# ctlab/metafast

Hardware: AMD Instinct MI355X
Metric: k-mers/s counted+graphed at k=31, 150 bp reads (higher is better)
Workload: dtype u64

## Files before the change

### metafast_amd/csrc/mf_skm.hip

```cpp
#include "mf_common.h"
#include "mf_count_dev.h"
#include <algorithm>
#include <memory>
#include <vector>

typedef ulonglong2 skm_rec;
typedef uint32_t skm_v4 __attribute__((ext_vector_type(4)));
#define SKM_LINE 4
#define SKM_QCAP 16
#define SKM_DIGIT_BITS 22
#define SKM_CT 512
#define SKM_NW (SKM_CT / 64)

__device__ __forceinline__ bool skm_rec_valid(const skm_rec &r) { return ((uint32_t)r.y & 63u) != 63u; }
__device__ __forceinline__ uint32_t skm_rec_n(const skm_rec &r) { return (uint32_t)r.y & 63u; }
__device__ __forceinline__ uint32_t skm_rec_digits(const skm_rec &r) { return (uint32_t)(r.y >> 6) & ((1u << SKM_DIGIT_BITS) - 1u); }

template <int K> struct skm_word {
    static constexpr int W = K - mf_skm_m(K) + 1;
    static constexpr int NM = 31 + W;
    static constexpr int RMAX = (MF_SKM_BASES - (K - 1)) < 20 ? (MF_SKM_BASES - (K - 1)) : 20;
    uint32_t D[4];
    uint32_t mh[32];
    uint32_t valid;
// ... 71 lines not shown
    const uint64_t b0 = w * 32;
    const uint4 *p = reinterpret_cast<const uint4 *>(bases + (b0 < n_bases ? b0 : 0));
    const bool in1 = b0 + 16 < n_bases;
    const uint4 c0 = p[0], c1 = p[in1 ? 1 : 0];
    S.D[0] = b0 < n_bases ? mf_dec16(c0) : 0u; S.D[1] = in1 ? mf_dec16(c1) : 0u;
    S.D[2] = skm_from_next_lane(S.D[0]); S.D[3] = skm_from_next_lane(S.D[1]);
    S.valid = m;
    static_assert(64 - M - 31 >= 16, "reversed words");
    const uint32_t R3 = skm_rc16(S.D[0]);
    const uint32_t R[4] = {0u, skm_from_next_lane(R3), skm_rc16(S.D[1]), R3};
    uint32_t hs[34];
#pragma unroll
    for (int i = 0; i < 32; i++) {
        const uint32_t f = skm_mmer_at<M>(S.D, i), r = skm_mmer_at<M>(R, 64 - M - i);
        hs[i] = mf_mmer_hash(f < r ? f : r, M);
    }
    constexpr int W = skm_word<K>::W;
    static_assert(W >= 3 && W <= 18, "window");
    static_assert(NM <= 64, "halo");
    auto min3 = [](uint32_t a, uint32_t b, uint32_t c) { const uint32_t m = a < b ? a : b; return m < c ? m : c; };
    hs[32] = skm_from_next_lane(hs[0]); hs[33] = skm_from_next_lane(hs[1]);
    uint32_t a[38];
#pragma unroll
    for (int i = 0; i < 32; i++) a[i] = min3(hs[i], hs[i + 1], hs[i + 2]);
    if (W >= 9) {
        uint32_t b[32 + 9];
#pragma unroll
        for (int i = 32; i < 38; i++) a[i] = skm_from_next_lane(a[i - 32]);
#pragma unroll
        for (int i = 0; i < 32; i++) b[i] = min3(a[i], a[i + 3], a[i + 6]);
#pragma unroll
        for (int i = 32; i < 32 + W - 9; i++) b[i] = skm_from_next_lane(b[i - 32]);
#pragma unroll
        for (int j = 0; j < 32; j++) S.mh[j] = b[j] < b[j + W - 9] ? b[j] : b[j + W - 9];
    } else {
        constexpr int D = W - 3 < 3 ? W - 3 : 3;
#pragma unroll
        for (int i = 32; i < 32 + W - 3; i++) a[i] = skm_from_next_lane(a[i - 32]);
#pragma unroll
        for (int j = 0; j < 32; j++) S.mh[j] = min3(a[j], a[j + D], a[j + W - 3]);
    }
    skm_cut_mask<K>(S, m);
}

__device__ __forceinline__ uint32_t skm_sel(uint32_t a, uint32_t b, unsigned long long m) {
    uint32_t r;
    asm("v_cndmask_b32 %0, %1, %2, %3" : "=v"(r) : "v"(a), "v"(b), "s"(m));
    return r;
}
template <int K>
__device__ __forceinline__ uint32_t skm_mh_at(const skm_word<K> &S, uint32_t s) {
    uint32_t a[16], b[8], c[4], d[2];
    const unsigned long long s0 = __ballot((s & 1u) != 0), s1 = __ballot((s & 2u) != 0), s2 = __ballot((s & 4u) != 0),
                             s3 = __ballot((s & 8u) != 0), s4 = __ballot((s & 16u) != 0);
#pragma unroll
    for (int i = 0; i < 16; i++) a[i] = skm_sel(S.mh[2 * i], S.mh[2 * i + 1], s0);
#pragma unroll
    for (int i = 0; i < 8; i++) b[i] = skm_sel(a[2 * i], a[2 * i + 1], s1);
#pragma unroll
    for (int i = 0; i < 4; i++) c[i] = skm_sel(b[2 * i], b[2 * i + 1], s2);
#pragma unroll
    for (int i = 0; i < 2; i++) d[i] = skm_sel(c[2 * i], c[2 * i + 1], s3);
    return skm_sel(d[0], d[1], s4);
}

template <int K>
__device__ __forceinline__ void skm_next_run(const skm_word<K> &S, uint32_t &cut, uint32_t &s, uint32_t &len) {
    s = (uint32_t)__builtin_ctz(cut);
    cut &= cut - 1u;
    const uint32_t stop = (cut | ~S.valid) & ~((2u << s) - 1u);
    const uint32_t e = stop ? (uint32_t)__builtin_ctz(stop) : 32u;
    len = e - s;
    if (len > (uint32_t)skm_word<K>::RMAX) { len = (uint32_t)skm_word<K>::RMAX; cut |= 1u << (s + len); }
}

template <int K>
__device__ __forceinline__ skm_rec skm_make_rec(const uint32_t (&D)[4], uint32_t s, uint32_t len, uint32_t digits, uint32_t D4 = 0u) {
    const uint32_t o = (2u * s) & 31u;
    const unsigned long long q = __ballot(s >= 16u);
    const uint32_t E0 = skm_sel(D[0], D[1], q), E1 = skm_sel(D[1], D[2], q), E2 = skm_sel(D[2], D[3], q), E3 = skm_sel(D[3], D4, q), E4 = skm_sel(D4, 0u, q);
    uint32_t T0 = E0, T1 = E1, T2 = E2, T3 = E3;
    if (o) {
        T0 = __builtin_amdgcn_alignbit(E0, E1, 32u - o);
        T1 = __builtin_amdgcn_alignbit(E1, E2, 32u - o);
        T2 = __builtin_amdgcn_alignbit(E2, E3, 32u - o);
        T3 = __builtin_amdgcn_alignbit(E3, E4, 32u - o);
    }
    static_assert(K >= 17 && K <= 32, "the first dword is kept whole");
    const int kb = 2 * (int)(len + K - 1);
    const uint64_t m01 = (uint64_t)((int64_t)0x8000000000000000ull >> ((kb < 64 ? kb : 64) - 1));
    const uint64_t m23 = ~(~0ull >> (kb > 64 ? kb - 64 : 0));
    T1 &= (uint32_t)m01; T2 &= (uint32_t)(m23 >> 32); T3 &= (uint32_t)m23;
    skm_rec r;
    r.x = ((uint64_t)T0 << 32) | T1;
    r.y = ((uint64_t)T2 << 32) | (uint64_t)(T3 & 0xF0000000u) | ((uint64_t)digits << 6) | (uint64_t)len;
    return r;
}
__device__ __forceinline__ void skm_route(uint32_t mh, int bits1, uint32_t &d1, uint32_t &digits) {
    const uint32_t ph = mf_remix32(mh);
    d1 = bits1 ? ph >> (32 - bits1) : 0u;
    digits = (bits1 ? (ph << bits1) : ph) >> (32 - SKM_DIGIT_BITS);
}

template <int K>
__global__ __launch_bounds__(1024) void k_skm_hist(const uint8_t *__restrict__ bases, uint64_t n_bases, const uint32_t *__restrict__ vmask,
                                                   uint64_t n_words, uint64_t words_per_block, int bits1,
                                                   uint32_t *__restrict__ blockhist, uint32_t *__restrict__ blockocc, int G, int stride,
                                                   uint32_t dlo, uint32_t dhi) {
    extern __shared__ __attribute__((aligned(16))) unsigned char smem[];
    const int nd = 1 << bits1;
    uint32_t *hist = reinterpret_cast<uint32_t *>(smem), *occ = hist + nd;
    for (int i = threadIdx.x; i < 2 * nd; i += blockDim.x) hist[i] = 0;
    __syncthreads();
    const uint64_t wlo = (uint64_t)blockIdx.x * words_per_block;
    const uint64_t whi = wlo + words_per_block < n_words ? wlo + words_per_block : n_words;
    for (uint64_t wb = wlo; wb < whi; wb += (uint64_t)blockDim.x * (uint64_t)stride) {
        const uint64_t w = wb + threadIdx.x;
        const uint32_t m = w < whi ? vmask[w] : 0u;
        if (__ballot(m != 0u) == 0ull) continue;
        skm_word<K> S;
        skm_scan_word<K>(S, bases, n_bases, w < n_words ? w : 0, m);
        uint32_t cut = S.cut;
        while (__ballot(cut != 0u) != 0ull) {
            if (cut) {
                uint32_t s, len, d1, digits;
                skm_next_run<K>(S, cut, s, len);
                skm_route(skm_mh_at<K>(S, s), bits1, d1, digits);
                if (d1 >= dlo && d1 < dhi) {
                    atomicAdd(&hist[d1], 1u);
                    if (blockocc) atomicAdd(&occ[d1], len);
                }
            }
        }
    }
    __syncthreads();
    for (int i = threadIdx.x; i < nd; i += blockDim.x) {
        blockhist[(size_t)i * G + blockIdx.x] = hist[i];
        if (blockocc) blockocc[(size_t)i * G + blockIdx.x] = occ[i];
    }
}

struct skm_stage {
    skm_rec *line;
    uint64_t *cur;
    uint64_t *q_pos;
    uint32_t *ctr;
    uint32_t *q_d;
    int nd;
};
__device__ __forceinline__ skm_stage skm_stage_carve(unsigned char *smem, int nd) {
    skm_stage L;
    L.nd = nd;
    L.line = reinterpret_cast<skm_rec *>(smem);
    L.cur = reinterpret_cast<uint64_t *>(L.line + (size_t)nd * SKM_LINE + 64);
    L.q_pos = L.cur + nd;
    L.ctr = reinterpret_cast<uint32_t *>(L.q_pos + 16 * SKM_QCAP);
    L.q_d = L.ctr + nd + 64;
    return L;
}
__host__ __device__ static inline size_t skm_stage_bytes(int nd) {
    return ((size_t)nd * SKM_LINE + 64) * 16 + (size_t)nd * 8 + 16 * SKM_QCAP * 8 + ((size_t)nd + 64) * 4 + 16 * SKM_QCAP * 4;
}
__device__ __forceinline__ void skm_lds_write4_add_rtn4(const uint32_t (&wa)[4], const skm_v4 (&wv)[4], const uint32_t (&a)[4],
                                                        const uint32_t (&inc)[4], uint32_t (&old)[4]) {
    asm volatile("ds_write_b128 %4, %8\n\tds_write_b128 %5, %9\n\tds_write_b128 %6, %10\n\tds_write_b128 %7, %11\n\t"
                 "ds_add_rtn_u32 %0, %12, %16\n\tds_add_rtn_u32 %1, %13, %17\n\tds_add_rtn_u32 %2, %14, %18\n\t"
                 "ds_add_rtn_u32 %3, %15, %19\n\ts_waitcnt lgkmcnt(0)"
                 : "=&v"(old[0]), "=&v"(old[1]), "=&v"(old[2]), "=&v"(old[3])
                 : "v"(wa[0]), "v"(wa[1]), "v"(wa[2]), "v"(wa[3]), "v"(wv[0]), "v"(wv[1]), "v"(wv[2]), "v"(wv[3]),
                   "v"(a[0]), "v"(a[1]), "v"(a[2]), "v"(a[3]), "v"(inc[0]), "v"(inc[1]), "v"(inc[2]), "v"(inc[3])
                 : "memory");
}
#define SKM_CH 256
#define SKM_NONE (~0ull)
struct skm_dyn {
    unsigned long long *gcur;
    const uint64_t *rend;
    unsigned int *overflow;
    uint64_t dump;
    unsigned long long *save;
};
template <bool DYN>
__device__ __forceinline__ uint64_t skm_take_line(const skm_stage &L, uint32_t dg, const skm_dyn &Dy) {
    uint64_t pos = L.cur[dg];
    if (DYN && (pos == SKM_NONE || (pos & (uint64_t)(SKM_CH - 1)) == 0ull)) {
        pos = atomicAdd(&Dy.gcur[dg], (unsigned long long)SKM_CH);
        if (pos + SKM_CH > Dy.rend[dg]) { atomicExch(Dy.overflow, 1u); pos = Dy.dump; }
    }
    L.cur[dg] = pos + SKM_LINE;
    return pos;
}
template <bool DYN = false>
__device__ __forceinline__ void skm_stage_insert(const skm_stage &L, skm_rec *__restrict__ out, const uint32_t (&d)[4],
                                                 const skm_rec (&rec)[4], bool (&pending)[4], const skm_dyn &Dy = skm_dyn()) {
    const uint32_t ctr0 = mf_lds_addr(L.ctr), line0 = mf_lds_addr(L.line);
    const uint32_t dummy_ctr = ctr0 + 4u * ((uint32_t)L.nd + (uint32_t)mf_lane());
    const uint32_t dummy_slot = line0 + 16u * ((uint32_t)L.nd * SKM_LINE + (uint32_t)mf_lane());
    skm_v4 wv[4];
#pragma unroll
    for (int b = 0; b < 4; b++) { wv[b].x = (uint32_t)rec[b].x; wv[b].y = (uint32_t)(rec[b].x >> 32); wv[b].z = (uint32_t)rec[b].y; wv[b].w = (uint32_t)(rec[b].y >> 32); }
    for (;;) {
        bool any = false;
#pragma unroll
        for (int b = 0; b < 4; b++) any |= pending[b];
        if (__ballot(any) == 0ull) break;
        uint32_t ca[4], w[4], inc[4], old[4], old2[4], wa[4];
        bool got[4];
#pragma unroll
        for (int b = 0; b < 4; b++) ca[b] = pending[b] ? ctr0 + 4u * d[b] : dummy_ctr;
        mf_lds_read4(ca, w);
#pragma unroll
        for (int b = 0; b < 4; b++) inc[b] = (pending[b] && (w[b] & 0xFFFFu) < (uint32_t)SKM_LINE) ? 1u : 0u;
        mf_lds_add_rtn4(ca, inc, old);
#pragma unroll
        for (int b = 0; b < 4; b++) {
            got[b] = inc[b] && (old[b] & 0xFFFFu) < (uint32_t)SKM_LINE;
            wa[b] = got[b] ? line0 + 16u * (d[b] * SKM_LINE + (old[b] & 0xFFFFu)) : dummy_slot;
            ca[b] = got[b] ? ctr0 + 4u * d[b] : dummy_ctr;
            inc[b] = got[b] ? 0x10000u : 0u;
        }
        skm_lds_write4_add_rtn4(wa, wv, ca, inc, old2);
        uint64_t *qpos = L.q_pos + (threadIdx.x >> 6) * SKM_QCAP;
        uint32_t *qd = L.q_d + (threadIdx.x >> 6) * SKM_QCAP;
        const uint64_t lt_mask = (1ull << mf_lane()) - 1ull;
#pragma unroll
        for (int b = 0; b < 4; b++) {
            const bool fl = got[b] && (old2[b] >> 16) == (uint32_t)(SKM_LINE - 1);
            const unsigned long long F = __ballot(fl);
            if (got[b]) pending[b] = false;
            if (F == 0ull) continue;
            const uint32_t n = (uint32_t)__popcll(F), qi = (uint32_t)__popcll(F & lt_mask);
            uint64_t mypos = 0;
            if (fl) mypos = skm_take_line<DYN>(L, d[b], Dy);
            for (uint32_t e0 = 0; e0 < n; e0 += SKM_QCAP) {
                if (fl && qi >= e0 && qi < e0 + SKM_QCAP) { qpos[qi - e0] = mypos; qd[qi - e0] = d[b]; }
                asm volatile("s_waitcnt lgkmcnt(0)" ::: "memory");
                const uint32_t e = e0 + ((uint32_t)mf_lane() >> 2), c = (uint32_t)mf_lane() & 3u;
                if (e < n) {
                    const uint32_t dd = qd[e - e0];
                    const uint64_t pp = qpos[e - e0];
                    const skm_rec v = L.line[dd * SKM_LINE + c];
                    out[pp + c] = v;
                    asm volatile("" ::: "memory");
                    if (c == 0) __hip_atomic_store(&L.ctr[dd], 0u, __ATOMIC_RELEASE, MF_WG);
                }
                asm volatile("s_waitcnt lgkmcnt(0)" ::: "memory");
            }
        }
        asm volatile("" ::: "memory");
        __builtin_amdgcn_wave_barrier();
    }
}
template <bool DYN = false>
__device__ __forceinline__ void skm_stage_flush_all(const skm_stage &L, skm_rec *__restrict__ out, int nd, const skm_dyn &Dy = skm_dyn()) {
    const skm_rec SENT = make_ulonglong2(~0ull, ~0ull);
    for (int d = threadIdx.x; d < nd; d += blockDim.x) {
        const uint32_t c = L.ctr[d] >> 16;
        if (c) {
            const uint64_t pos = skm_take_line<DYN>(L, (uint32_t)d, Dy);
            for (uint32_t s = 0; s < (uint32_t)SKM_LINE; s++) out[pos + s] = s < c ? L.line[d * SKM_LINE + s] : SENT;
            L.ctr[d] = 0;
        }
        if (DYN) {
            uint64_t pos = L.cur[d];
            if (Dy.save) Dy.save[(size_t)blockIdx.x * nd + d] = pos;
            else if (pos != SKM_NONE) for (; (pos & (uint64_t)(SKM_CH - 1)) != 0ull; pos++) out[pos] = SENT;
        }
    }
}
__global__ void k_skm_close_chunks(const unsigned long long *__restrict__ save, uint64_t n, uint64_t cap, skm_rec *__restrict__ out) {
    const uint64_t i = (uint64_t)blockIdx.x * blockDim.x + threadIdx.x;
    if (i >= n) return;
    uint64_t pos = save[i];
    if (pos == SKM_NONE || pos >= cap) return;
    const skm_rec SENT = make_ulonglong2(~0ull, ~0ull);
    for (; (pos & (uint64_t)(SKM_CH - 1)) != 0ull; pos++) out[pos] = SENT;
}

#define SKM_LCAP 384
#define SKM_FAST_WAVE_BYTES (64 * 16 + 64 * 8 + (SKM_LCAP + 1) * 8)
template <int K, bool DYN, bool FAST>
__global__ __launch_bounds__(1024) void k_skm_scatter(const uint8_t *__restrict__ bases, uint64_t n_bases, const uint32_t *__restrict__ vmask,
                                                      uint64_t n_words, uint64_t words_per_block, int bits1,
                                                      const uint64_t *__restrict__ blockstart, int G, skm_rec *__restrict__ out, skm_dyn Dy,
                                                      uint32_t dlo, uint32_t dhi) {
    extern __shared__ __attribute__((aligned(16))) unsigned char smem[];
    const int nd = 1 << bits1;
    skm_stage L = skm_stage_carve(smem, nd);
    if (DYN) Dy.dump += (uint64_t)blockIdx.x * SKM_CH;
    for (int i = threadIdx.x; i < nd; i += blockDim.x) {
        L.cur[i] = DYN ? (Dy.save ? (uint64_t)Dy.save[(size_t)blockIdx.x * nd + i] : SKM_NONE) : blockstart[(size_t)i * G + blockIdx.x];
        L.ctr[i] = 0;
    }
    if (threadIdx.x < 64) L.ctr[nd + threadIdx.x] = 0;
    __syncthreads();
    const uint32_t lane = (uint32_t)mf_lane();
    unsigned char *wbase = smem + ((skm_stage_bytes(nd) + 15) & ~(size_t)15) + (size_t)(threadIdx.x >> 6) * SKM_FAST_WAVE_BYTES;
    uint4 *pd = reinterpret_cast<uint4 *>(wbase);
    uint2 *pc = reinterpret_cast<uint2 *>(wbase + 64 * 16);
    uint2 *rl = reinterpret_cast<uint2 *>(wbase + 64 * 16 + 64 * 8);
    const uint64_t wlo = (uint64_t)blockIdx.x * words_per_block;
    const uint64_t whi = wlo + words_per_block < n_words ? wlo + words_per_block : n_words;
    const uint64_t wstep = (uint64_t)(blockDim.x >> 6) * 63u;
    for (uint64_t wb = wlo; wb < whi; wb += wstep) {
        const uint64_t w = wb + (uint64_t)(threadIdx.x >> 6) * 63u + lane;
        const uint32_t m = (lane < 63u && w < whi) ? vmask[w] : 0u;
        if (__ballot(m != 0u) == 0ull) continue;
        skm_word<K> S;
        skm_scan_word_halo<K>(S, bases, n_bases, w < n_words ? w : 0, m);
        uint32_t cut = S.cut;
        bool fast = FAST;
        uint32_t NR = 0, roff = 0, cutf = cut, ext = 0;
        if (FAST) {
            constexpr int R = skm_word<K>::RMAX;
            static_assert(R >= 16 && R <= 20, "run-length check");
            const uint32_t z = ~(cut | ~S.valid);
            const uint32_t z2 = z & (z >> 1), z4 = z2 & (z2 >> 2), z8 = z4 & (z4 >> 4), z16 = z8 & (z8 >> 8);
            const uint32_t zr = R == 16 ? z16 : (R == 17 ? (z16 & (z >> 16)) : (R == 18 ? (z16 & (z2 >> 16)) : (R == 19 ? (z16 & (z2 >> 16) & (z >> 18)) : (z16 & (z4 >> 16)))));
            const uint32_t pcut = skm_from_prev_lane(cut), pvalid = skm_from_prev_lane(S.valid), pm31 = skm_from_prev_lane(S.mh[31]);
            const bool cont = (S.valid & 1u) && (pvalid >> 31) && S.mh[0] == pm31;
            const uint32_t hstop = (cut & ~1u) | ~S.valid;
            const uint32_t h = hstop ? (uint32_t)__builtin_ctz(hstop) : 32u;
            const uint32_t tail = pcut ? (uint32_t)__builtin_clz(pcut) + 1u : 32u;
            constexpr uint32_t XMAX = 49 - K < R ? (uint32_t)(49 - K) : (uint32_t)R;
            uint32_t allowed = tail < (uint32_t)R ? (uint32_t)R - tail : 0u;
            if (allowed > XMAX) allowed = XMAX;
            ext = (DYN && cont) ? (h < allowed ? h : allowed) : 0u;
            cutf = ext ? ((cut & ~1u) | (ext < h ? (1u << ext) : 0u)) : cut;
            roff = mf_wave_excl_scan((uint32_t)__popc(cutf), &NR);
            fast = __ballot(zr != 0u) == 0ull && NR <= (uint32_t)SKM_LCAP;
        }
        if (FAST && fast) {
            pd[lane] = make_uint4(S.D[0], S.D[1], S.D[2], S.D[3]);
            pc[lane] = make_uint2(cutf | ~S.valid, ext);
            {
                const uint32_t l0 = mf_lds_addr(rl), dummy = l0 + 8u * (uint32_t)SKM_LCAP;
                uint32_t at = l0 + 8u * roff;
                const uint32_t tagl = lane << 5;
#pragma unroll
                for (int j = 0; j < 32; j++) {
                    const uint32_t bit = (cutf >> j) & 1u;
                    const uint32_t addr = bit ? at : dummy;
                    const uint32_t v1 = tagl | (uint32_t)j;
                    asm volatile("ds_write2_b32 %0, %1, %2 offset1:1" :: "v"(addr), "v"(S.mh[j]), "v"(v1) : "memory");
                    at += bit << 3;
                }
            }
            asm volatile("s_waitcnt lgkmcnt(0)" ::: "memory");
            __builtin_amdgcn_wave_barrier();
            for (uint32_t g0 = 0; g0 < NR; g0 += 256) {
                uint32_t d[4]; skm_rec rec[4]; bool pend[4];
#pragma unroll
                for (int b = 0; b < 4; b++) {
                    const uint32_t g = g0 + 64u * (uint32_t)b + lane;
                    pend[b] = g < NR;
                    const uint2 de = rl[pend[b] ? g : 0u];
                    const uint32_t src = (de.y >> 5) & 63u, s0 = de.y & 31u;
                    const uint4 Dw = pd[src]; const uint2 cv = pc[src];
                    const uint4 Dn = pd[(src + 1u) & 63u]; const uint2 cn = pc[(src + 1u) & 63u];
                    const uint32_t stop = cv.x & ~((2u << s0) - 1u);
                    const uint32_t e = stop ? (uint32_t)__builtin_ctz(stop) : 32u;
                    const uint32_t len = e - s0 + (e == 32u ? cn.y : 0u);
                    const uint32_t DD[4] = {Dw.x, Dw.y, Dw.z, Dw.w};
                    uint32_t digits;
                    skm_route(de.x, bits1, d[b], digits);
                    rec[b] = skm_make_rec<K>(DD, s0, len, digits, Dn.z);
                    if (!pend[b] || d[b] < dlo || d[b] >= dhi) { pend[b] = false; d[b] = 0; rec[b] = make_ulonglong2(~0ull, ~0ull); }
                }
                skm_stage_insert<DYN>(L, out, d, rec, pend, Dy);
            }
            asm volatile("s_waitcnt lgkmcnt(0)" ::: "memory");
            __builtin_amdgcn_wave_barrier();
            continue;
        }
        while (__ballot(cut != 0u) != 0ull) {
            uint32_t d[4]; skm_rec rec[4]; bool pend[4];
#pragma unroll
            for (int b = 0; b < 4; b++) {
                pend[b] = cut != 0u;
                d[b] = 0; rec[b] = make_ulonglong2(~0ull, ~0ull);
                if (pend[b]) {
                    uint32_t s, len, digits;
                    skm_next_run<K>(S, cut, s, len);
                    skm_route(skm_mh_at<K>(S, s), bits1, d[b], digits);
                    rec[b] = skm_make_rec<K>(S.D, s, len, digits);
                    if (d[b] < dlo || d[b] >= dhi) { pend[b] = false; d[b] = 0; }
                }
            }
            skm_stage_insert<DYN>(L, out, d, rec, pend, Dy);
        }
    }
    __syncthreads();
    skm_stage_flush_all<DYN>(L, out, nd, Dy);
}

__global__ void k_skm_region_sizes(const uint32_t *__restrict__ blockhist, int G, int nd, uint32_t scale, uint32_t *__restrict__ rsize,
                                   uint32_t dlo, uint32_t dhi) {
    const int d = blockIdx.x * blockDim.x + threadIdx.x;
    if (d >= nd) return;
    if ((uint32_t)d < dlo || (uint32_t)d >= dhi) { rsize[d] = 0; return; }
    uint64_t t = 0;
    for (int b = 0; b < G; b++) t += blockhist[(size_t)d * G + b];
    t *= scale;
    t += t / 16 + (uint64_t)G * SKM_CH + 8192;
    t = (t + SKM_CH - 1) & ~(uint64_t)(SKM_CH - 1);
    rsize[d] = t > 0xFFFFFF00ull ? 0xFFFFFF00u : (uint32_t)t;
}
__global__ void k_skm_dir_dyn(const uint64_t *__restrict__ rstart, const unsigned long long *__restrict__ gcur, int nd,
                              uint64_t *__restrict__ pstart, uint32_t *__restrict__ plen) {
    const int d = blockIdx.x * blockDim.x + threadIdx.x;
    if (d >= nd) return;
    pstart[d] = rstart[d];
    plen[d] = (uint32_t)(gcur[d] - rstart[d]);
}

__global__ void k_skm_dir(const uint64_t *__restrict__ blockstart, const uint32_t *__restrict__ blockocc, int G, int nd,
                          uint64_t *__restrict__ pstart, uint32_t *__restrict__ plen, uint32_t *__restrict__ pocc) {
    const int d = blockIdx.x * blockDim.x + threadIdx.x;
    if (d >= nd) return;
    const uint64_t s = blockstart[(size_t)d * G], e = blockstart[(size_t)(d + 1) * G];
    pstart[d] = s;
    plen[d] = (uint32_t)(e - s);
    if (blockocc) {
        uint64_t t = 0;
        for (int b = 0; b < G; b++) t += blockocc[(size_t)d * G + b];
        pocc[d] = t > 0xFFFFFFFFull ? 0xFFFFFFFFu : (uint32_t)t;
    }
}

__global__ __launch_bounds__(1024) void k_skm_split(const skm_rec *__restrict__ in, const uint64_t *__restrict__ pstart,
                                                    const uint32_t *__restrict__ plen, uint32_t np, int shift, int bits,
                                                    skm_rec *__restrict__ out, uint64_t *__restrict__ ostart, uint32_t *__restrict__ olen,
                                                    uint32_t *__restrict__ oocc, unsigned long long *__restrict__ n_valid, uint64_t rebase) {
    extern __shared__ __attribute__((aligned(16))) unsigned char smem[];
    __shared__ uint32_t scratch[17];
    const int nd = 1 << bits;
    const uint32_t dmask = (uint32_t)nd - 1u;
    skm_stage L = skm_stage_carve(smem, nd);
    uint32_t *occ = reinterpret_cast<uint32_t *>(L.line);
    const int ipt = (nd + (int)blockDim.x - 1) / (int)blockDim.x;
    for (uint32_t p = blockIdx.x; p < np; p += gridDim.x) {
        const uint64_t start = pstart[p];
        const uint32_t len = plen[p];
        const uint64_t obase = start - rebase + (uint64_t)p * (uint64_t)(SKM_LINE * nd);
        for (int i = threadIdx.x; i < nd; i += blockDim.x) { L.ctr[i] = 0; occ[i] = 0; }
        __syncthreads();
        const skm_rec *src = in + start;
        for (uint32_t jb = 0; jb < len; jb += 4 * blockDim.x) {
            skm_rec v[4];
#pragma unroll
            for (int u = 0; u < 4; u++) { const uint32_t j = jb + u * blockDim.x + threadIdx.x; v[u] = j < len ? src[j] : make_ulonglong2(~0ull, ~0ull); }
#pragma unroll
            for (int u = 0; u < 4; u++)
                if (skm_rec_valid(v[u])) {
                    const uint32_t dg = (skm_rec_digits(v[u]) >> shift) & dmask;
                    atomicAdd(&L.ctr[dg], 1u);
                    if (oocc) atomicAdd(&occ[dg], skm_rec_n(v[u]));
                }
        }
        __syncthreads();
        uint32_t mine = 0, raw = 0;
        const int b0 = threadIdx.x * ipt;
        for (int j = 0; j < ipt; j++) { const int b = b0 + j; if (b < nd) { mine += (L.ctr[b] + 3u) & ~3u; raw += L.ctr[b]; } }
        if (n_valid) {
            for (int dd = 32; dd >= 1; dd >>= 1) raw += __shfl_down(raw, dd, 64);
            if (mf_lane() == 0 && raw) atomicAdd(n_valid, (unsigned long long)raw);
        }
        uint32_t tot;
        uint32_t ex = mf_block_excl_scan(mine, scratch, &tot);
        for (int j = 0; j < ipt; j++) {
            const int b = b0 + j;
            if (b < nd) {
                const uint32_t c = (L.ctr[b] + 3u) & ~3u;
                L.cur[b] = obase + ex;
                ostart[(size_t)p * nd + b] = obase + ex;
                olen[(size_t)p * nd + b] = c;
                if (oocc) oocc[(size_t)p * nd + b] = occ[b];
                ex += c;
            }
        }
        __syncthreads();
        for (int i = threadIdx.x; i < nd; i += blockDim.x) L.ctr[i] = 0;
        if (threadIdx.x < 64) L.ctr[nd + threadIdx.x] = 0;
        __syncthreads();
        for (uint32_t jb = 0; jb < len; jb += 4 * blockDim.x) {
            skm_rec v[4]; uint32_t d[4]; bool pend[4];
#pragma unroll
            for (int u = 0; u < 4; u++) {
                const uint32_t j = jb + u * blockDim.x + threadIdx.x;
                v[u] = j < len ? src[j] : make_ulonglong2(~0ull, ~0ull);
                pend[u] = skm_rec_valid(v[u]);
                d[u] = pend[u] ? ((skm_rec_digits(v[u]) >> shift) & dmask) : 0u;
            }
            skm_stage_insert(L, out, d, v, pend);
        }
        __syncthreads();
        skm_stage_flush_all(L, out, nd);
        __syncthreads();
    }
}

#define SKM_MAX_PASSES 64
__device__ __forceinline__ uint32_t skm_pass_of(uint64_t key) {
    uint32_t g = ((uint32_t)(key >> 32) * 0xC2B2AE35u) ^ ((uint32_t)key * 0x27D4EB2Fu);
    g ^= g >> 15; g *= 0x165667B1u;
    return g >> 24;
}

#define C2_WG_PER_CU 2
#define C2_SLOTS 4096
#define C2_FILL 3400
#define C2_PASS_GROWTH 4u
#define C2_QN 128
#define C2_LH 64
#define C2_ITEMS 848
#define C2_W 2
#define DD_BITS 11
#define C2_DD 4
static constexpr size_t C2_LDS = (size_t)C2_SLOTS * 12 + (size_t)SKM_CT * 16 + (size_t)(SKM_CT / 64) * (C2_ITEMS * 2 + C2_QN * 8 + C2_QN * 2) + 2 * C2_LH * 4 + 48;
static_assert(C2_LDS <= 160 * 1024 / C2_WG_PER_CU, "workgroups per CU");

__device__ __forceinline__ uint32_t c2_swap_pairs(uint32_t x) {
    return ((x >> 1) & 0x55555555u) | ((x & 0x55555555u) << 1);
}
__device__ __forceinline__ uint32_t c2_slot(uint32_t hi, uint32_t lo) {
    uint32_t x = lo ^ __builtin_amdgcn_alignbit(hi, hi, 19);
    x ^= x >> 15;
    uint32_t t;
    asm("v_mul_u32_u24 %0, %1, %2" : "=v"(t) : "v"(x), "s"(0x9E3779u));
    return (t >> 11) & (uint32_t)(C2_SLOTS - 1);
}
struct c2_wave {
    uint32_t tk0, tc0, rb0, items0, qk0, qw0;
};
__device__ __forceinline__ unsigned long long c2_eq_u64(uint64_t a, uint64_t b) {
    unsigned long long m;
    asm("v_cmp_eq_u64_e64 %0, %1, %2" : "=s"(m) : "v"(a), "v"(b));
    return m;
}
__device__ __forceinline__ unsigned long long c2_lt_u32(uint32_t a, uint32_t b) {
    unsigned long long m;
    asm("v_cmp_lt_u32_e64 %0, %1, %2" : "=s"(m) : "v"(a), "v"(b));
    return m;
}
template <int U> __device__ __forceinline__ unsigned long long c2_gt(uint32_t a) {
    unsigned long long m;
    asm("v_cmp_lt_u32_e64 %0, %2, %1" : "=s"(m) : "v"(a), "n"(U));
    return m;
}
__device__ __forceinline__ void c2_barrier() { asm volatile("s_waitcnt lgkmcnt(0)\n\ts_barrier" ::: "memory"); }
__device__ __forceinline__ uint64_t c2_uniform64(uint64_t v) {
    return (uint64_t)(uint32_t)__builtin_amdgcn_readfirstlane((int)(uint32_t)v) | ((uint64_t)(uint32_t)__builtin_amdgcn_readfirstlane((int)(uint32_t)(v >> 32)) << 32);
}
__device__ __forceinline__ void c2_push64(unsigned long long m, uint32_t addr, uint64_t v) {
    unsigned long long save;
    asm volatile("s_mov_b64 %0, exec\n\ts_mov_b64 exec, %1\n\tds_write_b64 %2, %3\n\ts_mov_b64 exec, %0"
                 : "=&s"(save) : "s"(m), "v"(addr), "v"(v) : "memory");
}
__device__ __forceinline__ void c2_push16(unsigned long long m, uint32_t addr, uint32_t v) {
    unsigned long long save;
    asm volatile("s_mov_b64 %0, exec\n\ts_mov_b64 exec, %1\n\tds_write_b16 %2, %3\n\ts_mov_b64 exec, %0"
                 : "=&s"(save) : "s"(m), "v"(addr), "v"(v) : "memory");
}
__device__ __forceinline__ uint64_t c2_cas_m(unsigned long long m, uint32_t addr, uint64_t key) {
    unsigned long long save; uint64_t ret;
    asm volatile("s_mov_b64 %1, exec\n\ts_mov_b64 exec, %2\n\tds_cmpst_rtn_b64 %0, %3, %4, %5\n\ts_mov_b64 exec, %1\n\ts_waitcnt lgkmcnt(0)"
                 : "=&v"(ret), "=&s"(save) : "s"(m), "v"(addr), "v"(MF_EMPTY), "v"(key) : "memory");
    return ret;
}
__device__ __forceinline__ void c2_add_m(unsigned long long m, uint32_t addr, uint32_t one) {
    unsigned long long save;
    asm volatile("s_mov_b64 %0, exec\n\ts_mov_b64 exec, %1\n\tds_add_u32 %2, %3\n\ts_mov_b64 exec, %0"
                 : "=&s"(save) : "s"(m), "v"(addr), "v"(one) : "memory");
}
__device__ __forceinline__ uint32_t c2_lds_u32(const uint32_t *p) {
    uint32_t v;
    asm volatile("ds_read_b32 %0, %1\n\ts_waitcnt lgkmcnt(0)" : "=v"(v) : "v"(mf_lds_addr(p)) : "memory");
    return (uint32_t)__builtin_amdgcn_readfirstlane((int)v);
}
__device__ __forceinline__ void c2_drain(const c2_wave &L, uint32_t &qn, uint32_t &won_acc, uint32_t *part_over) {
    const uint32_t lane = (uint32_t)mf_lane();
    constexpr uint32_t mask = (uint32_t)(C2_SLOTS - 1);
    const uint32_t c = qn < 64u ? qn : 64u;
    qn -= c;
    unsigned long long pend = c2_lt_u32(lane, c);
    uint64_t key; uint32_t one;
    asm volatile("ds_read_b64 %0, %2\n\tds_read_u16 %1, %3\n\ts_waitcnt lgkmcnt(0)" : "=&v"(key), "=&v"(one) : "v"(L.qk0 + 8u * (qn + lane)), "v"(L.qw0 + 2u * (qn + lane)) : "memory");
    uint32_t s = (c2_slot((uint32_t)(key >> 32), (uint32_t)key) + 1u) & mask;
    for (uint32_t probes = 0; pend != 0ull; probes += 4) {
        if (probes >= 256u && ((probes & 255u) == 0u)) {
            if (probes > (uint32_t)C2_SLOTS) { if (lane == 0) *part_over = 1u; break; }
            if (c2_lds_u32(part_over)) break;
        }
        uint32_t a[4]; uint64_t v[4]; unsigned long long save;
#pragma unroll
        for (int j = 0; j < 4; j++) a[j] = L.tk0 + 8u * ((s + (uint32_t)j) & mask);
        asm volatile("s_mov_b64 %4, exec\n\ts_mov_b64 exec, %5\n\tds_read_b64 %0, %6\n\tds_read_b64 %1, %7\n\tds_read_b64 %2, %8\n\tds_read_b64 %3, %9\n\t"
                     "s_mov_b64 exec, %4\n\ts_waitcnt lgkmcnt(0)"
                     : "=&v"(v[0]), "=&v"(v[1]), "=&v"(v[2]), "=&v"(v[3]), "=&s"(save)
                     : "s"(pend), "v"(a[0]), "v"(a[1]), "v"(a[2]), "v"(a[3]) : "memory");
        unsigned long long eK[4], ev[4];
#pragma unroll
        for (int j = 0; j < 4; j++) { eK[j] = c2_eq_u64(v[j], key); ev[j] = eK[j] | c2_eq_u64(v[j], MF_EMPTY); }
        const unsigned long long any = pend & (ev[0] | ev[1] | ev[2] | ev[3]);
        uint32_t j = skm_sel(3u, 2u, ev[2]); j = skm_sel(j, 1u, ev[1]); j = skm_sel(j, 0u, ev[0]);
        const unsigned long long f0 = ev[0], f1 = ev[1] & ~ev[0], f2 = ev[2] & ~(ev[0] | ev[1]), f3 = ev[3] & ~(ev[0] | ev[1] | ev[2]);
        unsigned long long ok = pend & ((f0 & eK[0]) | (f1 & eK[1]) | (f2 & eK[2]) | (f3 & eK[3]));
        const unsigned long long need = any & ~ok;
        const uint32_t sj = (s + j) & mask;
        unsigned long long lost = 0ull;
        if (need != 0ull) {
            const uint64_t ret = c2_cas_m(need, L.tk0 + 8u * sj, key);
            const unsigned long long won = need & c2_eq_u64(ret, MF_EMPTY);
            ok |= won | (need & c2_eq_u64(ret, key));
            lost = need & ~ok;
            won_acc += (uint32_t)__popcll(won);
        }
        c2_add_m(ok, L.tc0 + 4u * sj, one);
        pend &= ~ok;
        s = skm_sel((s + 4u) & mask, (sj + 1u) & mask, lost);
    }
}

template <int K>
__device__ __forceinline__ void c2_step(const c2_wave &L, uint32_t i0, uint32_t &it, skm_v4 &W, uint32_t &it1, uint32_t &qn,
                                        uint32_t &won_acc, uint32_t *part_over, uint32_t P, uint32_t pass) {
    constexpr int sh = 64 - 2 * K;
    constexpr int nb = 2 * K - 34;
    const uint32_t lane = (uint32_t)mf_lane();
    const uint32_t nk = it & 3u;
    const uint32_t sa = it >> 10;
    unsigned long long q;
    asm("v_cmp_lt_u32_e64 %0, %2, %1" : "=s"(q) : "v"(it), "s"(0x7FFFu));
    const uint32_t A = skm_sel(W.y, W.x, q), B = skm_sel(W.z, W.y, q), C = skm_sel(W.w, W.z, q);
    const uint32_t hr = __builtin_amdgcn_alignbit(A, B, sa), lr = __builtin_amdgcn_alignbit(B, C, sa);
    uint32_t fh[2], fl[2], ch[2], cl[2];
// ... 1395 lines not shown
```

Baseline: 90.10 billion.

## Use exec-masked LDS ops instead of dummy slots in supermer staging

Replaces the dummy-address trick in the LDS staging insert with inline asm that sets the exec mask from ballots, so inactive lanes skip the ds_read/add/write entirely. The dummy counter and slot padding in shared memory are removed, and the run-list writer now uses an exec-masked carry-chain asm that writes only set bits. Wave-uniform word offsets are also hoisted into scalar registers via readfirstlane, and the flush step hits early-exit before the per-batch ballot loop. This cuts LDS traffic and bank conflicts on dummy addresses, at the cost of fragile hand-written asm and exec manipulation.

```diff
diff --git a/metafast_amd/csrc/mf_skm.hip b/metafast_amd/csrc/mf_skm.hip
--- a/metafast_amd/csrc/mf_skm.hip
+++ b/metafast_amd/csrc/mf_skm.hip
@@ -247,23 +247,51 @@
     skm_stage L;
     L.nd = nd;
     L.line = reinterpret_cast<skm_rec *>(smem);
-    L.cur = reinterpret_cast<uint64_t *>(L.line + (size_t)nd * SKM_LINE + 64);
+    L.cur = reinterpret_cast<uint64_t *>(L.line + (size_t)nd * SKM_LINE);
     L.q_pos = L.cur + nd;
     L.ctr = reinterpret_cast<uint32_t *>(L.q_pos + 16 * SKM_QCAP);
-    L.q_d = L.ctr + nd + 64;
+    L.q_d = L.ctr + nd;
     return L;
 }
 __host__ __device__ static inline size_t skm_stage_bytes(int nd) {
-    return ((size_t)nd * SKM_LINE + 64) * 16 + (size_t)nd * 8 + 16 * SKM_QCAP * 8 + ((size_t)nd + 64) * 4 + 16 * SKM_QCAP * 4;
-}
-__device__ __forceinline__ void skm_lds_write4_add_rtn4(const uint32_t (&wa)[4], const skm_v4 (&wv)[4], const uint32_t (&a)[4],
-                                                        const uint32_t (&inc)[4], uint32_t (&old)[4]) {
-    asm volatile("ds_write_b128 %4, %8\n\tds_write_b128 %5, %9\n\tds_write_b128 %6, %10\n\tds_write_b128 %7, %11\n\t"
-                 "ds_add_rtn_u32 %0, %12, %16\n\tds_add_rtn_u32 %1, %13, %17\n\tds_add_rtn_u32 %2, %14, %18\n\t"
-                 "ds_add_rtn_u32 %3, %15, %19\n\ts_waitcnt lgkmcnt(0)"
-                 : "=&v"(old[0]), "=&v"(old[1]), "=&v"(old[2]), "=&v"(old[3])
-                 : "v"(wa[0]), "v"(wa[1]), "v"(wa[2]), "v"(wa[3]), "v"(wv[0]), "v"(wv[1]), "v"(wv[2]), "v"(wv[3]),
-                   "v"(a[0]), "v"(a[1]), "v"(a[2]), "v"(a[3]), "v"(inc[0]), "v"(inc[1]), "v"(inc[2]), "v"(inc[3])
+    return (size_t)nd * SKM_LINE * 16 + (size_t)nd * 8 + 16 * SKM_QCAP * 8 + (size_t)nd * 4 + 16 * SKM_QCAP * 4;
+}
+__device__ __forceinline__ void skm_lds_read4_if(const unsigned long long (&m)[4], const uint32_t (&a)[4], uint32_t (&v)[4]) {
+    unsigned long long sv;
+    asm volatile("s_mov_b64 %4, exec\n\t"
+                 "s_mov_b64 exec, %5\n\tds_read_b32 %0, %9\n\t"
+                 "s_mov_b64 exec, %6\n\tds_read_b32 %1, %10\n\t"
+                 "s_mov_b64 exec, %7\n\tds_read_b32 %2, %11\n\t"
+                 "s_mov_b64 exec, %8\n\tds_read_b32 %3, %12\n\t"
+                 "s_mov_b64 exec, %4\n\ts_waitcnt lgkmcnt(0)"
+                 : "=&v"(v[0]), "=&v"(v[1]), "=&v"(v[2]), "=&v"(v[3]), "=&s"(sv)
+                 : "s"(m[0]), "s"(m[1]), "s"(m[2]), "s"(m[3]), "v"(a[0]), "v"(a[1]), "v"(a[2]), "v"(a[3])
+                 : "memory");
+}
+__device__ __forceinline__ void skm_lds_add_rtn4_if(const unsigned long long (&m)[4], const uint32_t (&a)[4], uint32_t inc, uint32_t (&old)[4]) {
+    unsigned long long sv;
+    asm volatile("s_mov_b64 %4, exec\n\t"
+                 "s_mov_b64 exec, %5\n\tds_add_rtn_u32 %0, %9, %13\n\t"
+                 "s_mov_b64 exec, %6\n\tds_add_rtn_u32 %1, %10, %13\n\t"
+                 "s_mov_b64 exec, %7\n\tds_add_rtn_u32 %2, %11, %13\n\t"
+                 "s_mov_b64 exec, %8\n\tds_add_rtn_u32 %3, %12, %13\n\t"
+                 "s_mov_b64 exec, %4\n\ts_waitcnt lgkmcnt(0)"
+                 : "=&v"(old[0]), "=&v"(old[1]), "=&v"(old[2]), "=&v"(old[3]), "=&s"(sv)
+                 : "s"(m[0]), "s"(m[1]), "s"(m[2]), "s"(m[3]), "v"(a[0]), "v"(a[1]), "v"(a[2]), "v"(a[3]), "v"(inc)
+                 : "memory");
+}
+__device__ __forceinline__ void skm_lds_write4_add_rtn4_if(const unsigned long long (&m)[4], const uint32_t (&wa)[4], const skm_v4 (&wv)[4],
+                                                           const uint32_t (&a)[4], uint32_t inc, uint32_t (&old)[4]) {
+    unsigned long long sv;
+    asm volatile("s_mov_b64 %4, exec\n\t"
+                 "s_mov_b64 exec, %5\n\tds_write_b128 %9, %13\n\tds_add_rtn_u32 %0, %17, %21\n\t"
+                 "s_mov_b64 exec, %6\n\tds_write_b128 %10, %14\n\tds_add_rtn_u32 %1, %18, %21\n\t"
+                 "s_mov_b64 exec, %7\n\tds_write_b128 %11, %15\n\tds_add_rtn_u32 %2, %19, %21\n\t"
+                 "s_mov_b64 exec, %8\n\tds_write_b128 %12, %16\n\tds_add_rtn_u32 %3, %20, %21\n\t"
+                 "s_mov_b64 exec, %4\n\ts_waitcnt lgkmcnt(0)"
+                 : "=&v"(old[0]), "=&v"(old[1]), "=&v"(old[2]), "=&v"(old[3]), "=&s"(sv)
+                 : "s"(m[0]), "s"(m[1]), "s"(m[2]), "s"(m[3]), "v"(wa[0]), "v"(wa[1]), "v"(wa[2]), "v"(wa[3]),
+                   "v"(wv[0]), "v"(wv[1]), "v"(wv[2]), "v"(wv[3]), "v"(a[0]), "v"(a[1]), "v"(a[2]), "v"(a[3]), "v"(inc)
                  : "memory");
 }
 #define SKM_CH 256
@@ -289,40 +317,47 @@
 __device__ __forceinline__ void skm_stage_insert(const skm_stage &L, skm_rec *__restrict__ out, const uint32_t (&d)[4],
                                                  const skm_rec (&rec)[4], bool (&pending)[4], const skm_dyn &Dy = skm_dyn()) {
     const uint32_t ctr0 = mf_lds_addr(L.ctr), line0 = mf_lds_addr(L.line);
-    const uint32_t dummy_ctr = ctr0 + 4u * ((uint32_t)L.nd + (uint32_t)mf_lane());
-    const uint32_t dummy_slot = line0 + 16u * ((uint32_t)L.nd * SKM_LINE + (uint32_t)mf_lane());
     skm_v4 wv[4];
-#pragma unroll
-    for (int b = 0; b < 4; b++) { wv[b].x = (uint32_t)rec[b].x; wv[b].y = (uint32_t)(rec[b].x >> 32); wv[b].z = (uint32_t)rec[b].y; wv[b].w = (uint32_t)(rec[b].y >> 32); }
+    uint32_t ca[4], la[4];
+#pragma unroll
+    for (int b = 0; b < 4; b++) {
+        wv[b].x = (uint32_t)rec[b].x; wv[b].y = (uint32_t)(rec[b].x >> 32); wv[b].z = (uint32_t)rec[b].y; wv[b].w = (uint32_t)(rec[b].y >> 32);
+        ca[b] = ctr0 + 4u * d[b];
+        la[b] = line0 + 16u * SKM_LINE * d[b];
+    }
     for (;;) {
-        bool any = false;
-#pragma unroll
-        for (int b = 0; b < 4; b++) any |= pending[b];
-        if (__ballot(any) == 0ull) break;
-        uint32_t ca[4], w[4], inc[4], old[4], old2[4], wa[4];
+        unsigned long long P[4], R[4], G[4];
+#pragma unroll
+        for (int b = 0; b < 4; b++) P[b] = __ballot(pending[b]);
+        if ((P[0] | P[1] | P[2] | P[3]) == 0ull) break;
+        uint32_t w[4], old[4], old2[4], wa[4];
         bool got[4];
-#pragma unroll
-        for (int b = 0; b < 4; b++) ca[b] = pending[b] ? ctr0 + 4u * d[b] : dummy_ctr;
-        mf_lds_read4(ca, w);
-#pragma unroll
-        for (int b = 0; b < 4; b++) inc[b] = (pending[b] && (w[b] & 0xFFFFu) < (uint32_t)SKM_LINE) ? 1u : 0u;
-        mf_lds_add_rtn4(ca, inc, old);
+        skm_lds_read4_if(P, ca, w);
+#pragma unroll
+        for (int b = 0; b < 4; b++) { got[b] = pending[b] && (w[b] & 0xFFFFu) < (uint32_t)SKM_LINE; R[b] = __ballot(got[b]); }
+        skm_lds_add_rtn4_if(R, ca, 1u, old);
 #pragma unroll
         for (int b = 0; b < 4; b++) {
-            got[b] = inc[b] && (old[b] & 0xFFFFu) < (uint32_t)SKM_LINE;
-            wa[b] = got[b] ? line0 + 16u * (d[b] * SKM_LINE + (old[b] & 0xFFFFu)) : dummy_slot;
-            ca[b] = got[b] ? ctr0 + 4u * d[b] : dummy_ctr;
-            inc[b] = got[b] ? 0x10000u : 0u;
-        }
-        skm_lds_write4_add_rtn4(wa, wv, ca, inc, old2);
+            got[b] = got[b] && (old[b] & 0xFFFFu) < (uint32_t)SKM_LINE;
+            wa[b] = la[b] + 16u * (old[b] & (uint32_t)(SKM_LINE - 1));
+            G[b] = __ballot(got[b]);
+        }
+        skm_lds_write4_add_rtn4_if(G, wa, wv, ca, 0x10000u, old2);
         uint64_t *qpos = L.q_pos + (threadIdx.x >> 6) * SKM_QCAP;
         uint32_t *qd = L.q_d + (threadIdx.x >> 6) * SKM_QCAP;
         const uint64_t lt_mask = (1ull << mf_lane()) - 1ull;
+        bool fl4[4], anyfl = false;
 #pragma unroll
         for (int b = 0; b < 4; b++) {
-            const bool fl = got[b] && (old2[b] >> 16) == (uint32_t)(SKM_LINE - 1);
+            fl4[b] = got[b] && (old2[b] >> 16) == (uint32_t)(SKM_LINE - 1);
+            anyfl |= fl4[b];
+            if (got[b]) pending[b] = false;
+        }
+        if (__ballot(anyfl) == 0ull) continue;
+#pragma unroll
+        for (int b = 0; b < 4; b++) {
+            const bool fl = fl4[b];
             const unsigned long long F = __ballot(fl);
-            if (got[b]) pending[b] = false;
             if (F == 0ull) continue;
             const uint32_t n = (uint32_t)__popcll(F), qi = (uint32_t)__popcll(F & lt_mask);
             uint64_t mypos = 0;
@@ -353,7 +388,11 @@
         const uint32_t c = L.ctr[d] >> 16;
         if (c) {
             const uint64_t pos = skm_take_line<DYN>(L, (uint32_t)d, Dy);
-            for (uint32_t s = 0; s < (uint32_t)SKM_LINE; s++) out[pos + s] = s < c ? L.line[d * SKM_LINE + s] : SENT;
+            for (uint32_t s = 0; s < (uint32_t)SKM_LINE; s++) {
+                skm_rec v = L.line[d * SKM_LINE + s];
+                if (s >= c) v = SENT;
+                out[pos + s] = v;
+            }
             L.ctr[d] = 0;
         }
         if (DYN) {
@@ -373,7 +412,28 @@
 }
 
 #define SKM_LCAP 384
-#define SKM_FAST_WAVE_BYTES (64 * 16 + 64 * 8 + (SKM_LCAP + 1) * 8)
+#define SKM_FAST_WAVE_BYTES (64 * 16 + 64 * 8 + SKM_LCAP * 8)
+template <int J0>
+__device__ __forceinline__ void skm_runlist8(uint32_t &c, uint32_t &at, uint32_t lane, uint32_t h0, uint32_t h1, uint32_t h2, uint32_t h3,
+                                             uint32_t h4, uint32_t h5, uint32_t h6, uint32_t h7) {
+    uint32_t t;
+    unsigned long long sv, m0, m1, m2, m3, m4, m5, m6, m7;
+#define SKM_RL_STEP(M, H, J) "s_mov_b64 exec, %[" M "]\n\tv_lshl_or_b32 %[t], %[lane], 5, %[" J "]\n\tds_write2_b32 %[at], %[" H "], %[t] offset1:1\n\tv_add_u32 %[at], 8, %[at]\n\t"
+    asm volatile("v_add_co_u32 %[c], %[m0], %[c], %[c]\n\tv_add_co_u32 %[c], %[m1], %[c], %[c]\n\t"
+                 "v_add_co_u32 %[c], %[m2], %[c], %[c]\n\tv_add_co_u32 %[c], %[m3], %[c], %[c]\n\t"
+                 "v_add_co_u32 %[c], %[m4], %[c], %[c]\n\tv_add_co_u32 %[c], %[m5], %[c], %[c]\n\t"
+                 "v_add_co_u32 %[c], %[m6], %[c], %[c]\n\tv_add_co_u32 %[c], %[m7], %[c], %[c]\n\t"
+                 "s_mov_b64 %[sv], exec\n\t"
+                 SKM_RL_STEP("m0", "h0", "j0") SKM_RL_STEP("m1", "h1", "j1") SKM_RL_STEP("m2", "h2", "j2") SKM_RL_STEP("m3", "h3", "j3")
+                 SKM_RL_STEP("m4", "h4", "j4") SKM_RL_STEP("m5", "h5", "j5") SKM_RL_STEP("m6", "h6", "j6") SKM_RL_STEP("m7", "h7", "j7")
+                 "s_mov_b64 exec, %[sv]"
+                 : [c] "+v"(c), [at] "+v"(at), [t] "=&v"(t), [sv] "=&s"(sv), [m0] "=&s"(m0), [m1] "=&s"(m1), [m2] "=&s"(m2), [m3] "=&s"(m3),
+                   [m4] "=&s"(m4), [m5] "=&s"(m5), [m6] "=&s"(m6), [m7] "=&s"(m7)
+                 : [lane] "v"(lane), [h0] "v"(h0), [h1] "v"(h1), [h2] "v"(h2), [h3] "v"(h3), [h4] "v"(h4), [h5] "v"(h5), [h6] "v"(h6), [h7] "v"(h7),
+                   [j0] "i"(J0), [j1] "i"(J0 + 1), [j2] "i"(J0 + 2), [j3] "i"(J0 + 3), [j4] "i"(J0 + 4), [j5] "i"(J0 + 5), [j6] "i"(J0 + 6), [j7] "i"(J0 + 7)
+                 : "memory");
+#undef SKM_RL_STEP
+}
 template <int K, bool DYN, bool FAST>
 __global__ __launch_bounds__(1024) void k_skm_scatter(const uint8_t *__restrict__ bases, uint64_t n_bases, const uint32_t *__restrict__ vmask,
                                                       uint64_t n_words, uint64_t words_per_block, int bits1,
@@ -387,7 +447,6 @@
         L.cur[i] = DYN ? (Dy.save ? (uint64_t)Dy.save[(size_t)blockIdx.x * nd + i] : SKM_NONE) : blockstart[(size_t)i * G + blockIdx.x];
         L.ctr[i] = 0;
     }
-    if (threadIdx.x < 64) L.ctr[nd + threadIdx.x] = 0;
     __syncthreads();
     const uint32_t lane = (uint32_t)mf_lane();
     unsigned char *wbase = smem + ((skm_stage_bytes(nd) + 15) & ~(size_t)15) + (size_t)(threadIdx.x >> 6) * SKM_FAST_WAVE_BYTES;
@@ -396,9 +455,13 @@
     uint2 *rl = reinterpret_cast<uint2 *>(wbase + 64 * 16 + 64 * 8);
     const uint64_t wlo = (uint64_t)blockIdx.x * words_per_block;
     const uint64_t whi = wlo + words_per_block < n_words ? wlo + words_per_block : n_words;
-    const uint64_t wstep = (uint64_t)(blockDim.x >> 6) * 63u;
+    const uint64_t wstep = (uint64_t)(uint32_t)__builtin_amdgcn_readfirstlane((int)(blockDim.x >> 6)) * 63u;
+    const uint64_t wave0 = (uint64_t)(uint32_t)__builtin_amdgcn_readfirstlane((int)(threadIdx.x >> 6)) * 63u;
     for (uint64_t wb = wlo; wb < whi; wb += wstep) {
-        const uint64_t w = wb + (uint64_t)(threadIdx.x >> 6) * 63u + lane;
+        uint32_t wlo32 = (uint32_t)__builtin_amdgcn_readfirstlane((int)(uint32_t)(wb + wave0));
+        uint32_t whi32 = (uint32_t)__builtin_amdgcn_readfirstlane((int)(uint32_t)((wb + wave0) >> 32));
+        asm("" : "+s"(wlo32), "+s"(whi32));
+        const uint64_t w = (((uint64_t)whi32 << 32) | wlo32) + lane;
         const uint32_t m = (lane < 63u && w < whi) ? vmask[w] : 0u;
         if (__ballot(m != 0u) == 0ull) continue;
         skm_word<K> S;
@@ -429,17 +492,11 @@
             pd[lane] = make_uint4(S.D[0], S.D[1], S.D[2], S.D[3]);
             pc[lane] = make_uint2(cutf | ~S.valid, ext);
             {
-                const uint32_t l0 = mf_lds_addr(rl), dummy = l0 + 8u * (uint32_t)SKM_LCAP;
-                uint32_t at = l0 + 8u * roff;
-                const uint32_t tagl = lane << 5;
-#pragma unroll
-                for (int j = 0; j < 32; j++) {
-                    const uint32_t bit = (cutf >> j) & 1u;
-                    const uint32_t addr = bit ? at : dummy;
-                    const uint32_t v1 = tagl | (uint32_t)j;
-                    asm volatile("ds_write2_b32 %0, %1, %2 offset1:1" :: "v"(addr), "v"(S.mh[j]), "v"(v1) : "memory");
-                    at += bit << 3;
-                }
+                uint32_t at = mf_lds_addr(rl) + 8u * roff, c = __brev(cutf);
+                skm_runlist8<0>(c, at, lane, S.mh[0], S.mh[1], S.mh[2], S.mh[3], S.mh[4], S.mh[5], S.mh[6], S.mh[7]);
+                skm_runlist8<8>(c, at, lane, S.mh[8], S.mh[9], S.mh[10], S.mh[11], S.mh[12], S.mh[13], S.mh[14], S.mh[15]);
+                skm_runlist8<16>(c, at, lane, S.mh[16], S.mh[17], S.mh[18], S.mh[19], S.mh[20], S.mh[21], S.mh[22], S.mh[23]);
+                skm_runlist8<24>(c, at, lane, S.mh[24], S.mh[25], S.mh[26], S.mh[27], S.mh[28], S.mh[29], S.mh[30], S.mh[31]);
             }
             asm volatile("s_waitcnt lgkmcnt(0)" ::: "memory");
             __builtin_amdgcn_wave_barrier();
@@ -460,7 +517,7 @@
                     uint32_t digits;
                     skm_route(de.x, bits1, d[b], digits);
                     rec[b] = skm_make_rec<K>(DD, s0, len, digits, Dn.z);
-                    if (!pend[b] || d[b] < dlo || d[b] >= dhi) { pend[b] = false; d[b] = 0; rec[b] = make_ulonglong2(~0ull, ~0ull); }
+                    if (d[b] < dlo || d[b] >= dhi) pend[b] = false;
                 }
                 skm_stage_insert<DYN>(L, out, d, rec, pend, Dy);
             }
@@ -576,7 +633,6 @@
         }
         __syncthreads();
         for (int i = threadIdx.x; i < nd; i += blockDim.x) L.ctr[i] = 0;
-        if (threadIdx.x < 64) L.ctr[nd + threadIdx.x] = 0;
         __syncthreads();
         for (uint32_t jb = 0; jb < len; jb += 4 * blockDim.x) {
             skm_rec v[4]; uint32_t d[4]; bool pend[4];
```

Measured after the change: 91.63 billion (median of 6 runs). +1.7%, better.
